# citiususc/BigSeqKit

Hardware: AMD Instinct MI355X
Metric: M records/s + GB/s (vs HBM roofline) on 100GB FASTQ stats (higher is better)
Workload: dtype u8; 1 GPU; bigseqkit stats on 100.0 GB synthetic FASTQ-150 (BASELINE C2: 315457413 records x 317 B), HBM-resident, 1 record-aligned shard(s); command=stats, records=315457413, bytes=99999999921, seed=42

## Files before the change

bigseqkit_amd/_lib.py:

```python
import ctypes as C
import os

_HERE = os.path.dirname(os.path.abspath(__file__))
LIB_PATH = os.environ.get("BSK_LIB", os.path.join(_HERE, "lib", "libbsk.so"))

if not os.path.exists(LIB_PATH):
    raise ImportError(
        f"libbsk.so not found at {LIB_PATH}: build it with ./build.sh "
        "(hipcc --offload-arch=gfx950); bigseqkit_amd has no CPU fallback")



def _preload_hip_runtime():
    import importlib.util
    try:
        spec = importlib.util.find_spec("torch")
    except Exception:
        spec = None
    if spec and spec.origin:
        cand = os.path.join(os.path.dirname(spec.origin), "lib", "libamdhip64.so")
        if os.path.exists(cand):
            try:
                C.CDLL(cand, mode=C.RTLD_GLOBAL)
            except OSError:
# ... 144 lines not shown
    "bsk_event_record": (_i, [_vp, _vp]),
    "bsk_event_elapsed_ms": (_i, [_vp, _vp, _p(C.c_float)]),
    "bsk_event_destroy": (_i, [_vp]),
    "bsk_selftest_regex_find": (_i, [C.c_char_p, C.c_char_p, _sz, _sz, _p(C.c_uint32), _p(C.c_uint32)]),
    "bsk_store_open": (_i, [C.c_char_p, _i, _p(_vp)]),
    "bsk_store_error": (C.c_char_p, [_vp]),
    "bsk_store_put": (_i, [_vp, _vp, _u64, _vp]),
    "bsk_store_put_host": (_i, [_vp, _u64, _vp, _sz]),
    "bsk_store_close": (_i, [_vp, _p(_u64)]),
    "bsk_run_to_store": (_i, [_vp, _vp, _sz, _i, _i64, _vp, _u64, _p(_u64), _p(_u64)]),
    "bsk_profile_enable": (_i, [_vp, _i]),
    "bsk_profile_read": (_i, [_vp, C.c_char_p, _p(C.c_double), _p(_u64)]),
    "bsk_profile_reset": (_i, [_vp]),
    "bsk_profile_dump": (_i, [_vp, C.c_char_p, _sz]),
    "bsk_selftest_scan": (_i, [_i, _p(C.c_uint32), _p(C.c_uint32)]),
    "bsk_selftest_rmdup_keys": (_i, [_vp, _p(_u64), _p(_u64), _sz, _p(_sz)]),
    "bsk_selftest_stream_read": (_i, [_vp, _sz, _i, _i, _p(C.c_float)]),
}

for _name, (_res, _args) in SIGNATURES.items():
    _f = getattr(lib, _name)
    _f.restype = _res
    _f.argtypes = _args


class BskError(RuntimeError):
    def __init__(self, code, message):
        super().__init__(message)
        self.code = code

# ... 7 lines not shown
```

bigseqkit_amd/csrc/anchor_wave_dev.hpp:

```cpp
#pragma once
#include <hip/hip_runtime.h>

#include <cstdint>

#include "anchor.hpp"

namespace bsk {
namespace wave_anchor {

__device__ __forceinline__ uint32_t first_eq16(const uint4& v, uint32_t rep) {
    const uint32_t w[4] = {v.x ^ rep, v.y ^ rep, v.z ^ rep, v.w ^ rep};
    uint32_t pos = 16u;
#pragma unroll
    for (int d = 3; d >= 0; --d) {
        const uint32_t x = w[d];
        const uint32_t z = ~(((x & 0x7F7F7F7Fu) + 0x7F7F7F7Fu) | x | 0x7F7F7F7Fu);
        if (z) pos = 4u * (uint32_t)d + (((uint32_t)__ffs((int)z) - 1u) >> 3);
    }
    return pos;
}

__device__ __forceinline__ uint64_t find_byte(const uint8_t* __restrict__ buf, uint64_t n, uint64_t from, uint8_t c) {
    const uint32_t lane = threadIdx.x & 63u;
    const uint32_t rep = 0x01010101u * c;
// ... 79 lines not shown
    if (e1 > s0 && buf[s0] == '+') return false;
    const uint64_t p0 = e1 + 1;
    if (p0 >= n || buf[p0] != '+') return false;
    const uint64_t e2 = find_byte(buf, n, p0, '\n');
    if (e2 >= n) return false;
    const uint64_t q0 = e2 + 1;
    const uint64_t e3 = find_byte(buf, n, q0, '\n');
    if (e3 - q0 != e1 - s0) return false;
    if (e3 + 1 < n) {
        const uint8_t c = buf[e3 + 1];
        if (c != '@' && c != '\n') return false;
    }
    return true;
}

__device__ __forceinline__ uint64_t find_fastq_start(const uint8_t* buf, uint64_t n, uint64_t from, uint64_t limit) {
    if (from >= n) return n;
    if (from == 0 && fastq_record_at(buf, n, 0)) return 0;
    uint64_t j = from == 0 ? find_byte(buf, n, 0, '\n') : find_byte(buf, n, from - 1, '\n');
    while (j < n) {
        if (fastq_record_at(buf, n, j + 1)) return j + 1;
        if (j >= limit) return ANCHOR_NONE;
        j = find_byte(buf, n, j + 1, '\n');
    }
    return n;
}

__device__ __forceinline__ uint64_t fastq_range_start(const uint8_t* buf, uint64_t n, uint64_t from) {
    const uint64_t a = find_fastq_start(buf, n, from, from + ANCHOR_SEARCH_BYTES);
    return a == ANCHOR_NONE ? from : a;
}

__device__ __forceinline__ uint64_t effective_end(const uint8_t* __restrict__ buf, uint64_t n) {
    const uint32_t lane = threadIdx.x & 63u;
    uint64_t k = 0;
    while (k < n) {
        const uint64_t left = n - k;
        const bool nl = lane < left && buf[left - 1u - lane] == '\n';
        const uint64_t other = ~__ballot(nl);
        const uint32_t run = other ? (uint32_t)__ffsll((long long)other) - 1u : 64u;
        k += run;
        if (run < 64u) break;
    }
    if (k > n) k = n;
    if (k == n) return 0;
// ... 6 lines not shown
```

bigseqkit_amd/csrc/capi.cpp:

```cpp
#include <hip/hip_runtime_api.h>

#include <algorithm>
#include <cstdio>
#include <cstdlib>
#include <cstring>
#include <new>
#include <optional>

#include "../../include/bsk.h"
#include "anchor.hpp"
#include "ctx.hpp"
#include "ops_host.hpp"
#include "ops_host_internal.hpp"
#include "ops_sample.hpp"
#include "ops_segcopy.hpp"
#include "stats_host.hpp"
#include "stream_stats.hpp"
#include "regex_vm.hpp"
#include "synth.hpp"

namespace bsk {
hipError_t launch_synth(int kind, uint64_t seed, unsigned flags, uint64_t first_record, uint8_t* dst, uint64_t n,
                        hipStream_t st);
}
// ... 398 lines not shown
    return BSK_OK;
}

static int stats_run_device(bsk_ctx* c, const uint8_t* d_buf, size_t n, int format, uint64_t* d_vec, hipStream_t st) {
    const bool fastq = format == BSK_FORMAT_FASTQ;
    const bool all = c->opts.b("All");
    const bool variant = fastq ? c->stats_a_dense : c->tune.is("stats_fasta", "events");
    const int per_cu = stats_max_blocks_per_cu(fastq, all, c->use_dpp, variant);
    const int blocks = std::max(1, c->num_cus * per_cu);
    const uint64_t waves = (uint64_t)blocks * 4;
    const uint64_t nr = pick_nranges(n, waves, c->min_range_bytes, (int)c->tune.num("ranges_per_wave"));
    const uint32_t nranges = (uint32_t)nr;
    uint64_t chunk = (n + nranges - 1) / nranges;
    chunk = (chunk + 15) & ~(uint64_t)15;
    const bool self_anchor = fastq && !all && c->use_dpp && !c->tune.is("stats_prep", "pass");
    uint32_t tickets = nranges, nsplit = nranges;
    if (self_anchor) {
        chunk = (chunk + 63) & ~(uint64_t)63;
        const uint64_t tail = nranges / 16, small = chunk / 4;
        const uint64_t floor_bytes = std::max<uint64_t>(c->min_range_bytes, (uint64_t)c->tune.num("stats_tail", 192 << 10));
        if (tail && small >= floor_bytes && !c->tune.is("stats_tail", "uniform") && (uint64_t)(nranges - tail) * chunk < n) {
            nsplit = (uint32_t)(nranges - tail);
            tickets = nsplit + (uint32_t)((n - (uint64_t)nsplit * chunk + small - 1) / small);
        }
    } else {
        int rc = ensure_range_arrays(c, nranges);
        if (rc != BSK_OK) return rc;
    }
    const uint64_t need = n / c->hist_cap + 1024;
    if (need > c->overflow_cap) {
        uint64_t* nb = nullptr;
        HIP_TRY(c, hipMalloc((void**)&nb, need * sizeof(uint64_t)));
        if (c->d_overflow) {
            HIP_TRY(c, hipMemcpyAsync(nb, c->d_overflow, c->overflow_cap * sizeof(uint64_t), hipMemcpyDeviceToDevice, st));
            HIP_TRY(c, hipStreamSynchronize(st));
            HIP_TRY(c, hipFree(c->d_overflow));
        }
        c->d_overflow = nb;
        c->overflow_cap = need;
// ... 26 lines not shown
    uint32_t* queue = self_anchor ? reinterpret_cast<uint32_t*>(c->d_ctl + bsk_ctx::CTL_STATS_QUEUE) : range_queue(c, nranges);
    D.r_head = D.r_tail = nullptr;
    D.r_flags = nullptr;
    if (!fastq) {
        if (nranges > c->rng_cap || !c->d_rng) {
            if (c->d_rng) HIP_TRY(c, hipFree(c->d_rng));
            c->d_rng = nullptr;
            HIP_TRY(c, hipMalloc((void**)&c->d_rng, (size_t)nranges * 20 + 64));
            c->rng_cap = nranges;
        }
        D.r_head = c->d_rng;
        D.r_tail = c->d_rng + nranges;
        D.r_flags = reinterpret_cast<uint32_t*>(c->d_rng + 2 * (size_t)nranges);
        HIP_TRY(c, hipMemsetAsync(c->d_rng, 0, (size_t)nranges * 20, st));
    }
    if (!self_anchor) {
        Timed t(c, "k_prep", st);
        HIP_TRY(c, launch_prep(fastq, d_buf, n, chunk, nranges, anchors, queue, st, !fastq,
                               fastq ? nullptr : c->d_anchors + (size_t)nranges + 2));
    }
    {
        Timed t(c, "k_stats", st);
        HIP_TRY(c, launch_stats(fastq, all, c->use_dpp, blocks, d_buf, n, anchors, tickets, queue, D, st, variant,
                                !fastq ? chunk : 0, self_anchor ? chunk : 0, nsplit));
    }
    if (!fastq) HIP_TRY(c, launch_stats_stitch(nranges, D, st));
    if (all && (int)gap_letters.size() > MAX_GAP_LETTERS) {
        const int rci = build_index(c, d_buf, n, format, st);
        if (rci != BSK_OK) return rci;
        uint32_t set[8] = {0, 0, 0, 0, 0, 0, 0, 0};
        for (char ch : gap_letters) set[(uint8_t)ch >> 5] |= 1u << ((uint8_t)ch & 31u);
        HIP_TRY(c, launch_gap_set_count(d_buf, c->table, set, fastq, D.vec + 2, st));
    }
    return BSK_OK;
}

static int stage_shard(bsk_ctx* c, const void* shard, size_t n, int on_device, hipStream_t st, const uint8_t** d);

int bsk_stats_run(bsk_ctx* c, const void* shard, size_t n, int on_device, int format, int64_t pid, void* d_vec,
                  void* stream) {
// ... 972 lines not shown
        HIP_TRY(nullptr, hipEventRecord(a, nullptr));
        HIP_TRY(nullptr, launch_stream_read(blocks, (const uint8_t*)d_buf, n, chunk, (uint32_t)nr, d, d + 1, nullptr));
        HIP_TRY(nullptr, hipEventRecord(b, nullptr));
        HIP_TRY(nullptr, hipEventSynchronize(b));
        float ms = 0;
        HIP_TRY(nullptr, hipEventElapsedTime(&ms, a, b));
        if (r > 0) total += ms;
    }
    *avg_ms = total / reps;
    hipEventDestroy(a);
    hipEventDestroy(b);
    hipFree(d);
    return BSK_OK;
}

int bsk_selftest_scan(int use_dpp, const uint32_t* in64, uint32_t* out64) {
    uint32_t *d_in = nullptr, *d_out = nullptr;
    HIP_TRY(nullptr, hipMalloc((void**)&d_in, 64 * 4));
    HIP_TRY(nullptr, hipMalloc((void**)&d_out, 64 * 4));
    HIP_TRY(nullptr, hipMemcpy(d_in, in64, 64 * 4, hipMemcpyHostToDevice));
    HIP_TRY(nullptr, launch_scan_selftest(use_dpp != 0, d_in, d_out, nullptr));
    HIP_TRY(nullptr, hipMemcpy(out64, d_out, 64 * 4, hipMemcpyDeviceToHost));
    hipFree(d_in);
    hipFree(d_out);
    return BSK_OK;
}

int bsk_selftest_regex_find(const char* expr, const uint8_t* text, size_t n, size_t from, uint32_t* caps4, uint32_t* ngroups) {
    try {
        const VmProgram P = compile_vm(expr ? expr : "");
// ... 10 lines not shown
```

bigseqkit_amd/csrc/stream_stats.hip:

```cpp
#include <hip/hip_runtime.h>

#include <algorithm>
#include <cstdint>

#include "anchor.hpp"
#include "anchor_wave_dev.hpp"
#include "index.hpp"
#include "stream_core_dev.hpp"
#include "stream_fasta2_dev.hpp"
#include "stream_stats.hpp"

namespace bsk {

namespace {

using namespace stream;

constexpr int BIG_SLOTS = 64;
constexpr uint32_t BIG_EMPTY = 0xFFFFFFFFu;

__device__ __forceinline__ void add_big(uint32_t len, uint32_t c, uint32_t* s_hist, const StatsDev& D) {
    uint32_t* keys = s_hist + LDS_HIST;
    uint32_t* cnts = keys + BIG_SLOTS;
    const uint32_t slot = (len * 2654435761u) >> 26;
// ... 279 lines not shown
                any_event = true;
            }
        }
    }
};

#ifndef BSK_STATS_WAVES
#define BSK_STATS_WAVES 7
#endif
#ifndef BSK_STATS_WAVES_ALL
#define BSK_STATS_WAVES_ALL 5
#endif
#ifndef BSK_STATS_WAVES_FQ
#define BSK_STATS_WAVES_FQ 6
#endif
#if BSK_STATS_WAVES
#ifndef BSK_STATS_WAVES_FA_ALL
#define BSK_STATS_WAVES_FA_ALL 5
#endif
#define BSK_STATS_ATTR __attribute__((amdgpu_waves_per_eu((ALL && FASTQ) ? BSK_STATS_WAVES_ALL : (FASTQ ? BSK_STATS_WAVES_FQ : ((ALL && ROLES_T) ? BSK_STATS_WAVES_FA_ALL : BSK_STATS_WAVES)), 8)))
#else
#define BSK_STATS_ATTR
#endif

template <bool FASTQ, bool ALL, bool DPP, bool ROLES_T = true>
__global__ __launch_bounds__(WAVES_PER_BLOCK * WAVE) BSK_STATS_ATTR void k_stats(const uint8_t* __restrict__ buf, uint64_t n,
                                                                   const uint64_t* __restrict__ anchors,
                                                                   uint32_t nranges, uint32_t* __restrict__ queue,
                                                                   StatsDev D, uint64_t chunk, uint32_t nsplit) {
    __shared__ uint32_t s_hist[LDS_HIST + 2 * BIG_SLOTS];
    constexpr bool ROLES = FASTQ && ALL && ROLES_T;
    constexpr bool SALL = ALL && !ROLES;
    constexpr int WINDOW = (FASTQ && !SALL) ? 256 : CAP;
    constexpr bool F2 = !FASTQ && ROLES_T;
    __shared__ Lds<FASTQ, SALL, F2 ? 4 : WINDOW> s_l[F2 ? 1 : WAVES_PER_BLOCK];
    __shared__ LdsF2T<F2 && ALL> s_f2[F2 ? WAVES_PER_BLOCK : 1];
    for (int i = threadIdx.x; i < LDS_HIST + 2 * BIG_SLOTS; i += blockDim.x)
        s_hist[i] = (i >= LDS_HIST && i < LDS_HIST + BIG_SLOTS) ? BIG_EMPTY : 0u;
    __syncthreads();

    const int lane = threadIdx.x & 63;
    const int wave = threadIdx.x >> 6;
    Lds<FASTQ, SALL, F2 ? 4 : WINDOW>& L = s_l[F2 ? 0 : wave];
    StatsSinkT<ROLES> sink;
    sink.s_hist = s_hist;
    sink.D = D;
    constexpr bool SELF = FASTQ && !ALL && DPP;
    const bool self_anchor = SELF && anchors == nullptr;
    const uint64_t n_eff = self_anchor ? wave_anchor::effective_end(buf, n) : anchors[nranges];
    uint64_t w20 = 0, w30 = 0, wgap = 0;
    for (;;) {
        uint32_t r = 0;
        if (lane == 0) r = atomicAdd(queue, 1u);
        r = wave_first(r);
        if (r >= nranges) break;
        uint64_t rs = 0, re = n_eff;
        if (self_anchor) {
            if constexpr (SELF) {
#pragma nounroll
                for (uint32_t k = 0; k < 2u; ++k) {
                    const uint32_t t = r + k;
                    if (t == 0u || t >= nranges) continue;
                    const uint64_t from = t <= nsplit ? (uint64_t)t * chunk : (uint64_t)nsplit * chunk + (uint64_t)(t - nsplit) * (chunk >> 2);
                    uint32_t flo = (uint32_t)from, fhi = (uint32_t)(from >> 32);
                    asm volatile("" : "+v"(flo), "+v"(fhi));
                    const uint64_t av = wave_anchor::fastq_range_start(buf, n, ((uint64_t)fhi << 32) | flo);
                    const uint64_t a = ((uint64_t)wave_first((uint32_t)(av >> 32)) << 32) | wave_first((uint32_t)av);
                    if (k == 0u) rs = a;
                    else re = a;
                }
            }
        } else {
            rs = anchors[r];
            re = anchors[r + 1];
        }
        rs = rs < n_eff ? rs : n_eff;
        re = re < n_eff ? re : n_eff;
        if (rs >= re) {
            if constexpr (!FASTQ && ALL) {
                if (chunk && r > 0u) {
                    const uint64_t lo = (uint64_t)r * chunk, hi = lo + chunk < n_eff ? lo + chunk : n_eff;
                    if (lo < hi) {
                        uint64_t cnt = 0;
                        for (uint64_t i = lo + (uint64_t)lane * 16u; i < hi; i += 64u * 16u) {
                            const uint4 v = load16(buf, hi, i);
                            for (int k = 0; k < D.pred.ngap; ++k) {
                                const uint32_t rep = D.pred.gap_rep[k];
                                if (rep == 0u && i + 16u > hi) continue;
                                cnt += popc4(zero_bytes(v.x ^ rep), zero_bytes(v.y ^ rep), zero_bytes(v.z ^ rep), zero_bytes(v.w ^ rep));
                            }
                        }
                        cnt = wave_sum_u64(cnt);
// ... 19 lines not shown
                sink.rgap = 0; sink.rsub = 0;
            }
            (void)L;
        } else {
            stream_range<FASTQ, SALL, DPP>(L, buf, n, rs, re, re == n_eff, D.pred, sink, skip_from, count_resume);
        }
        if constexpr (!FASTQ) sink.template end_range<ALL>();
        if constexpr (ROLES) {
            const uint64_t s20 = wave_sum_u64(sink.rq20), s30 = wave_sum_u64(sink.rq30), sgap = wave_sum_u64(sink.rgap);
            w20 += ((uint64_t)wave_first((uint32_t)(s20 >> 32)) << 32) | wave_first((uint32_t)s20);
            w30 += ((uint64_t)wave_first((uint32_t)(s30 >> 32)) << 32) | wave_first((uint32_t)s30);
            wgap += ((uint64_t)wave_first((uint32_t)(sgap >> 32)) << 32) | wave_first((uint32_t)sgap);
            sink.rq20 = sink.rq30 = sink.rgap = 0;
        }
    }
    if (self_anchor && lane == 0) {
        if (atomicAdd(queue + 1, 1u) == gridDim.x * (uint32_t)WAVES_PER_BLOCK - 1u) {
            atomicExch(queue + 1, 0u);
            atomicExch(queue, 0u);
        }
    }
    const uint64_t q20 = ROLES ? w20 : wave_sum_u64(sink.q20), q30 = ROLES ? w30 : wave_sum_u64(sink.q30),
                   gap = ROLES ? wgap : wave_sum_u64(sink.gap);
    const uint64_t nrec = wave_sum_u64(sink.nrec), sumlen = wave_sum_u64(sink.sumlen);
    const uint32_t err = wave_or_u32(sink.err);
    if (lane == 0) {
        if (q20) atomicAdd((unsigned long long*)&D.vec[0], (unsigned long long)q20);
        if (q30) atomicAdd((unsigned long long*)&D.vec[1], (unsigned long long)q30);
        if (gap) atomicAdd((unsigned long long*)&D.vec[2], (unsigned long long)gap);
        if (nrec) atomicAdd((unsigned long long*)&D.vec[3], (unsigned long long)nrec);
// ... 19 lines not shown
    if (r > nranges) return;
    if (r == 0) {
        if (lane0) { anchors[0] = 0; *queue = 0; }
        return;
    }
    if (r == nranges) {
        if (lane0) anchors[nranges] = effective_end(buf, n);
        return;
    }
    const uint64_t from = (uint64_t)r * chunk;
    if (!FASTQ && line_mode == 2) {
        const uint64_t a = wave_anchor::find_line_start_within(buf, n, from, from + chunk);
        if (lane0) anchors[r] = a;
        return;
    }
    const uint64_t a = FASTQ ? wave_anchor::fastq_range_start(buf, n, from)
                             : (line_mode ? wave_anchor::find_line_start(buf, n, from) : wave_anchor::find_fasta_start(buf, n, from));
    if (lane0) anchors[r] = a == ANCHOR_NONE ? from : a;
}

__global__ __launch_bounds__(256) void k_prep_fill(const uint64_t* __restrict__ raw, uint32_t nranges, uint64_t* __restrict__ anchors) {
    const uint32_t r = blockIdx.x * blockDim.x + threadIdx.x;
    if (r > nranges) return;
    uint32_t j = r;
    while (j < nranges && raw[j] == ANCHOR_NONE) ++j;
    anchors[r] = raw[j];
}

__global__ __launch_bounds__(256) void k_stats_stitch(uint32_t nranges, StatsDev D) {
    __shared__ uint32_t s_hist[LDS_HIST + 2 * BIG_SLOTS];
    __shared__ unsigned long long s_nrec, s_sum;
// ... 58 lines not shown
                if (idx + 16 <= re) {
                    const uint4 v = *reinterpret_cast<const uint4*>(buf + idx);
                    acc ^= v.x ^ v.y ^ v.z ^ v.w;
                }
            }
        }
    }
    if (acc == 0x9E3779B9u) sink[0] = acc;
}

template <bool DPP>
__global__ void k_scan_selftest(const uint32_t* in, uint32_t* out) {
    out[threadIdx.x] = wave_incl_scan<DPP>(in[threadIdx.x]);
}

}

hipError_t launch_prep(bool fastq, const uint8_t* buf, uint64_t n, uint64_t chunk, uint32_t nranges,
                       uint64_t* anchors, uint32_t* queue, hipStream_t st, bool line_mode, uint64_t* raw) {
    const int threads = 256;
    const int blocks = (int)(((uint64_t)nranges + 1 + 3) / 4);
    if (fastq) hipLaunchKernelGGL(k_prep<true>, dim3(blocks), dim3(threads), 0, st, buf, n, chunk, nranges, anchors, queue, 0);
    else if (line_mode && raw) {
        hipLaunchKernelGGL(k_prep<false>, dim3(blocks), dim3(threads), 0, st, buf, n, chunk, nranges, raw, queue, 2);
        hipLaunchKernelGGL(k_prep_fill, dim3((nranges + 1 + 255) / 256), dim3(256), 0, st, (const uint64_t*)raw, nranges, anchors);
    } else hipLaunchKernelGGL(k_prep<false>, dim3(blocks), dim3(threads), 0, st, buf, n, chunk, nranges, anchors, queue, line_mode ? 1 : 0);
    return hipGetLastError();
}

__global__ __launch_bounds__(1024) void k_stats_pack(const uint64_t* __restrict__ vec, uint32_t cap, const uint64_t* __restrict__ status,
// ... 52 lines not shown
    if (t.n == 0) return hipSuccess;
    GapSet S;
    for (int i = 0; i < 8; ++i) S.w[i] = set[i];
    const uint64_t blocks = std::min<uint64_t>((t.n + 3) / 4, 256ull * 32ull);
    hipLaunchKernelGGL(k_gap_set_count, dim3((unsigned)blocks), dim3(256), 0, st, buf, t, S, fastq ? 1 : 0, (unsigned long long*)gap_slot);
    return hipGetLastError();
}

hipError_t launch_stats_stitch(uint32_t nranges, const StatsDev& D, hipStream_t st) {
    hipLaunchKernelGGL(k_stats_stitch, dim3((nranges + 255u) / 256u), dim3(256), 0, st, nranges, D);
    return hipGetLastError();
}

template <bool FASTQ, bool ALL, bool ROLES_T = true>
static hipError_t launch_stats_t(bool dpp, int blocks, const uint8_t* buf, uint64_t n, const uint64_t* anchors,
                                 uint32_t nranges, uint32_t* queue, const StatsDev& D, hipStream_t st, uint64_t chunk, uint32_t nsplit = 0) {
    const dim3 b(WAVES_PER_BLOCK * WAVE);
    if (dpp) hipLaunchKernelGGL((k_stats<FASTQ, ALL, true, ROLES_T>), dim3(blocks), b, 0, st, buf, n, anchors, nranges, queue, D, chunk, nsplit);
    else hipLaunchKernelGGL((k_stats<FASTQ, ALL, false, ROLES_T>), dim3(blocks), b, 0, st, buf, n, anchors, nranges, queue, D, chunk, nsplit);
    return hipGetLastError();
}

hipError_t launch_stats(bool fastq, bool all, bool dpp, int blocks, const uint8_t* buf, uint64_t n,
                        const uint64_t* anchors, uint32_t nranges, uint32_t* queue, const StatsDev& D,
                        hipStream_t st, bool a_dense, uint64_t skip_chunk, uint64_t fq_chunk, uint32_t fq_nsplit) {
    if (fastq && all && a_dense) return launch_stats_t<true, true, false>(dpp, blocks, buf, n, anchors, nranges, queue, D, st, fq_chunk, fq_nsplit);
    if (fastq) return all ? launch_stats_t<true, true>(dpp, blocks, buf, n, anchors, nranges, queue, D, st, fq_chunk, fq_nsplit)
                          : launch_stats_t<true, false>(dpp, blocks, buf, n, anchors, nranges, queue, D, st, fq_chunk, fq_nsplit);
    if (all) return a_dense ? launch_stats_t<false, true, false>(dpp, blocks, buf, n, anchors, nranges, queue, D, st, skip_chunk)
                            : launch_stats_t<false, true>(dpp, blocks, buf, n, anchors, nranges, queue, D, st, skip_chunk);
    return a_dense ? launch_stats_t<false, false, false>(dpp, blocks, buf, n, anchors, nranges, queue, D, st, skip_chunk)
                   : launch_stats_t<false, false>(dpp, blocks, buf, n, anchors, nranges, queue, D, st, skip_chunk);
}

int stats_max_blocks_per_cu(bool fastq, bool all, bool dpp, bool a_dense) {
    const void* f = nullptr;
#define BSK_PICK(FQ, AL, RO)                                                            \
    f = dpp ? (const void*)k_stats<FQ, AL, true, RO> : (const void*)k_stats<FQ, AL, false, RO>;
    if (fastq && all && a_dense) { BSK_PICK(true, true, false) }
    else if (fastq && all) { BSK_PICK(true, true, true) }
    else if (fastq) { BSK_PICK(true, false, true) }
    else if (all && a_dense) { BSK_PICK(false, true, false) }
    else if (all) { BSK_PICK(false, true, true) }
    else if (a_dense) { BSK_PICK(false, false, false) }
    else { BSK_PICK(false, false, true) }
#undef BSK_PICK
    return blocks_per_cu(f, WAVES_PER_BLOCK * WAVE);
}

hipError_t launch_stream_read(int blocks, const uint8_t* buf, uint64_t n, uint64_t chunk, uint32_t nranges,
                              uint32_t* queue, uint32_t* sink, hipStream_t st) {
    hipLaunchKernelGGL(k_stream_read, dim3(blocks), dim3(WAVES_PER_BLOCK * WAVE), 0, st, buf, n, chunk, nranges, queue,
                       sink);
    return hipGetLastError();
}

hipError_t launch_scan_selftest(bool dpp, const uint32_t* in, uint32_t* out, hipStream_t st) {
    if (dpp) hipLaunchKernelGGL(k_scan_selftest<true>, dim3(1), dim3(64), 0, st, in, out);
    else hipLaunchKernelGGL(k_scan_selftest<false>, dim3(1), dim3(64), 0, st, in, out);
    return hipGetLastError();
}

}
```

bigseqkit_amd/csrc/stream_stats.hpp:

```cpp
#pragma once
#include <hip/hip_runtime_api.h>

#include <cstdint>

namespace bsk {

constexpr int STATS_HDR = 8;
constexpr int MAX_GAP_LETTERS = 8;

constexpr uint32_t ERR_BAD_HEADER = 1u;
constexpr uint32_t ERR_BAD_PLUS = 2u;
constexpr uint32_t ERR_LEN_MISMATCH = 4u;
constexpr uint32_t ERR_TRUNCATED = 8u;
constexpr uint32_t ERR_ANCHOR = 16u;
constexpr uint32_t ERR_LINE_TOO_LONG = 32u;
constexpr uint32_t ERR_CAPACITY = 64u;

inline int blocks_per_cu(const void* kernel, int threads) {
    int nb = 0;
    if (hipOccupancyMaxActiveBlocksPerMultiprocessor(&nb, kernel, threads, 0) != hipSuccess || nb < 1) nb = 1;
    return nb;
}

struct PredConsts {
// ... 16 lines not shown
};

constexpr uint32_t RF_VISITED = 1u, RF_HAS_HEADER = 2u, RF_HEAD_CLOSED = 4u, RF_TAIL_OPEN = 8u;
constexpr uint32_t RF_MID = 16u, RF_SKIP_SEQ = 32u;

hipError_t launch_prep(bool fastq, const uint8_t* buf, uint64_t n, uint64_t chunk, uint32_t nranges,
                       uint64_t* anchors, uint32_t* queue, hipStream_t st, bool line_mode = false, uint64_t* raw = nullptr);
hipError_t launch_stats_stitch(uint32_t nranges, const StatsDev& D, hipStream_t st);
struct RecordTable;
hipError_t launch_gap_set_count(const uint8_t* buf, const RecordTable& t, const uint32_t (&set)[8], bool fastq, uint64_t* gap_slot,
                                hipStream_t st);
hipError_t launch_stats_pack(const uint64_t* vec, uint32_t cap, const uint64_t* status, uint64_t* pack, uint32_t kbins, hipStream_t st);
hipError_t launch_stats(bool fastq, bool all, bool dpp, int blocks, const uint8_t* buf, uint64_t n,
                        const uint64_t* anchors, uint32_t nranges, uint32_t* queue, const StatsDev& D,
                        hipStream_t st, bool a_dense = false, uint64_t skip_chunk = 0,
                        uint64_t fq_chunk = 0, uint32_t fq_nsplit = 0);
int stats_max_blocks_per_cu(bool fastq, bool all, bool dpp, bool a_dense = false);
hipError_t launch_stream_read(int blocks, const uint8_t* buf, uint64_t n, uint64_t chunk, uint32_t nranges,
                              uint32_t* queue, uint32_t* sink, hipStream_t st);
hipError_t launch_scan_selftest(bool dpp, const uint32_t* in, uint32_t* out, hipStream_t st);

}
```

include/bsk.h:

```cpp
#ifndef BSK_H
#define BSK_H

#include <stddef.h>
#include <stdint.h>

#ifdef __cplusplus
extern "C" {
#endif

#define BSK_OK 0
#define BSK_ERR_INVALID_ARG 1
#define BSK_ERR_OPTS 2
#define BSK_ERR_FORMAT 3
#define BSK_ERR_UNSUPPORTED 4
#define BSK_ERR_HIP 5
#define BSK_ERR_NO_DEVICE 6
#define BSK_ERR_CAPACITY 7
#define BSK_ERR_OVERFLOW_EXCHANGE 8

#define BSK_FORMAT_FASTA 0
#define BSK_FORMAT_FASTQ 1

typedef struct bsk_ctx bsk_ctx;

// ... 202 lines not shown
uint64_t bsk_synth_offset(int kind, uint64_t record);
int bsk_synth_host(int kind, uint64_t seed, unsigned flags, uint64_t first_record, uint8_t* dst, size_t n);
int bsk_synth_device(int kind, uint64_t seed, unsigned flags, uint64_t first_record, void* d_dst, size_t n, int device,
                     void* stream);

int bsk_event_create(void** ev);
int bsk_event_record(void* ev, void* stream);
int bsk_event_elapsed_ms(void* start, void* stop, float* ms);
int bsk_event_destroy(void* ev);
int bsk_profile_enable(bsk_ctx* ctx, int on);
int bsk_profile_read(bsk_ctx* ctx, const char* kernel, double* total_ms, uint64_t* launches);
int bsk_profile_reset(bsk_ctx* ctx);
int bsk_profile_dump(bsk_ctx* ctx, char* buf, size_t cap);

int bsk_selftest_scan(int use_dpp, const uint32_t* in64, uint32_t* out64);
int bsk_selftest_rmdup_keys(bsk_ctx* ctx, uint64_t* k1, uint64_t* k2, size_t cap, size_t* n_out);
int bsk_selftest_stream_read(const void* d_buf, size_t n, int reps, int blocks_per_cu, float* avg_ms);

#ifdef __cplusplus
}
#endif
#endif
```

Before: 20950 M records/s.

## Use geometric multi-level tail ranges and windowed FASTQ anchor search in stats

Replaces the single split of the stats work queue (uniform chunks plus one small-chunk tail) with up to eight levels of halving range sizes, each ticket mapped to its boundary through a per-level table passed as a kernel argument. Self-anchoring FASTQ range starts now load a 2 KB window per wave once, build newline/@/+ bitmasks across lanes, and validate record starts from those masks, falling back to the byte scan only when the window is inconclusive. The aim is better tail load balance and fewer dependent global loads when finding record boundaries. In exchange the kernel carries more argument state and branching, and adds optional clock instrumentation and selftests.

Result: no change. 20910 M records/s (-0.2%).

```diff
diff --git a/bigseqkit_amd/_lib.py b/bigseqkit_amd/_lib.py
--- a/bigseqkit_amd/_lib.py
+++ b/bigseqkit_amd/_lib.py
@@ -182,6 +182,9 @@
     "bsk_profile_reset": (_i, [_vp]),
     "bsk_profile_dump": (_i, [_vp, C.c_char_p, _sz]),
     "bsk_selftest_scan": (_i, [_i, _p(C.c_uint32), _p(C.c_uint32)]),
+    "bsk_selftest_fastq_range_start": (_i, [C.c_void_p, C.c_size_t, _p(C.c_uint64), C.c_size_t, C.c_size_t, _p(C.c_uint64)]),
+    "bsk_selftest_fastq_range_start_host": (_i, [C.c_void_p, C.c_size_t, _p(C.c_uint64), C.c_size_t, _i, _p(C.c_uint64)]),
+    "bsk_selftest_stats_levels": (_i, [C.c_uint64, C.c_uint64, C.c_uint64, _i, C.c_uint64, _p(C.c_uint64), _p(C.c_uint64)]),
     "bsk_selftest_rmdup_keys": (_i, [_vp, _p(_u64), _p(_u64), _sz, _p(_sz)]),
     "bsk_selftest_stream_read": (_i, [_vp, _sz, _i, _i, _p(C.c_float)]),
 }
diff --git a/bigseqkit_amd/csrc/anchor_wave_dev.hpp b/bigseqkit_amd/csrc/anchor_wave_dev.hpp
--- a/bigseqkit_amd/csrc/anchor_wave_dev.hpp
+++ b/bigseqkit_amd/csrc/anchor_wave_dev.hpp
@@ -117,10 +117,8 @@
     return true;
 }
 
-__device__ __forceinline__ uint64_t find_fastq_start(const uint8_t* buf, uint64_t n, uint64_t from, uint64_t limit) {
-    if (from >= n) return n;
-    if (from == 0 && fastq_record_at(buf, n, 0)) return 0;
-    uint64_t j = from == 0 ? find_byte(buf, n, 0, '\n') : find_byte(buf, n, from - 1, '\n');
+__device__ __forceinline__ uint64_t find_fastq_start_from(const uint8_t* buf, uint64_t n, uint64_t x, uint64_t limit) {
+    uint64_t j = find_byte(buf, n, x, '\n');
     while (j < n) {
         if (fastq_record_at(buf, n, j + 1)) return j + 1;
         if (j >= limit) return ANCHOR_NONE;
@@ -129,9 +127,143 @@
     return n;
 }
 
+__device__ __forceinline__ uint64_t find_fastq_start(const uint8_t* buf, uint64_t n, uint64_t from, uint64_t limit) {
+    if (from >= n) return n;
+    if (from == 0 && fastq_record_at(buf, n, 0)) return 0;
+    return find_fastq_start_from(buf, n, from == 0 ? 0 : from - 1, limit);
+}
+
 __device__ __forceinline__ uint64_t fastq_range_start(const uint8_t* buf, uint64_t n, uint64_t from) {
     const uint64_t a = find_fastq_start(buf, n, from, from + ANCHOR_SEARCH_BYTES);
     return a == ANCHOR_NONE ? from : a;
+}
+
+constexpr uint32_t WIN_BYTES = 2048u;
+constexpr uint32_t WIN_NONE = 0xFFFFFFFFu;
+
+struct FqWindow { uint32_t nl, at, pl; };
+
+__device__ __forceinline__ uint64_t fastq_window_base(const uint8_t* buf, uint64_t from) {
+    const uint64_t x = from - 1u;
+    const uint64_t off = (uint64_t)(reinterpret_cast<uintptr_t>(buf + x) & 15u);
+    return x >= off ? x - off : x;
+}
+
+__device__ __forceinline__ uint4 window_load16(const uint8_t* __restrict__ buf, uint64_t n, uint64_t i) {
+    uint4 v = make_uint4(0u, 0u, 0u, 0u);
+    if (i + 16u <= n) __builtin_memcpy(&v, buf + i, 16);
+    else if (i < n) {
+        uint32_t w[4] = {0u, 0u, 0u, 0u};
+        for (uint32_t b = 0; b < 16u && i + b < n; ++b) w[b >> 2] |= (uint32_t)buf[i + b] << ((b & 3u) * 8u);
+        v = make_uint4(w[0], w[1], w[2], w[3]);
+    }
+    return v;
+}
+
+__device__ __forceinline__ void fastq_window_load(const uint8_t* __restrict__ buf, uint64_t n, uint64_t w0, uint4& a, uint4& b) {
+    const uint64_t i = w0 + (uint64_t)(threadIdx.x & 63u) * 32u;
+    a = window_load16(buf, n, i);
+    b = window_load16(buf, n, i + 16u);
+}
+
+__device__ __forceinline__ uint32_t window_eq16(const uint4& v, uint32_t rep) {
+    const uint32_t w[4] = {v.x ^ rep, v.y ^ rep, v.z ^ rep, v.w ^ rep};
+    uint32_t m = 0u;
+#pragma unroll
+    for (int d = 0; d < 4; ++d) {
+        const uint32_t x = w[d];
+        const uint32_t z = ~(((x & 0x7F7F7F7Fu) + 0x7F7F7F7Fu) | x | 0x7F7F7F7Fu);
+        m |= (((z >> 7) | (z >> 14) | (z >> 21) | (z >> 28)) & 0xFu) << (4 * d);
+    }
+    return m;
+}
+
+__device__ __forceinline__ FqWindow fastq_window_masks(const uint4& a, const uint4& b) {
+    FqWindow W;
+    W.nl = window_eq16(a, 0x0A0A0A0Au) | (window_eq16(b, 0x0A0A0A0Au) << 16);
+    W.at = window_eq16(a, 0x40404040u) | (window_eq16(b, 0x40404040u) << 16);
+    W.pl = window_eq16(a, 0x2B2B2B2Bu) | (window_eq16(b, 0x2B2B2B2Bu) << 16);
+    return W;
+}
+
+__device__ __forceinline__ uint32_t window_next(uint32_t m, uint64_t any, uint32_t x) {
+    if (x >= WIN_BYTES) return WIN_NONE;
+    const uint32_t l = x >> 5;
+    const uint32_t w = (uint32_t)__builtin_amdgcn_readlane((int)m, (int)l) & (~0u << (x & 31u));
+    if (w) return (l << 5) + (uint32_t)__ffs((int)w) - 1u;
+    const uint64_t rest = l >= 63u ? 0ull : any & (~0ull << (l + 1u));
+    if (!rest) return WIN_NONE;
+    const uint32_t l2 = (uint32_t)__ffsll((long long)rest) - 1u;
+    return (l2 << 5) + (uint32_t)__ffs(__builtin_amdgcn_readlane((int)m, (int)l2)) - 1u;
+}
+__device__ __forceinline__ bool window_bit(uint32_t m, uint32_t x) {
+    return (((uint32_t)__builtin_amdgcn_readlane((int)m, (int)(x >> 5)) >> (x & 31u)) & 1u) != 0u;
+}
+
+__device__ __forceinline__ int fastq_window_record_at(const FqWindow& W, uint64_t any_nl, uint32_t p, uint32_t end) {
+    const bool reach = end != WIN_NONE;
+    const int open = reach ? 0 : -1;
+    if (reach && p >= end) return 0;
+    if (p >= WIN_BYTES) return -1;
+    if (!window_bit(W.at, p)) return 0;
+    const uint32_t e0 = window_next(W.nl, any_nl, p);
+    if (e0 == WIN_NONE) return open;
+    const uint32_t s0 = e0 + 1u;
+    const uint32_t e1 = window_next(W.nl, any_nl, s0);
+    if (e1 == WIN_NONE) return open;
+    if (e1 > s0 && window_bit(W.pl, s0)) return 0;
+    const uint32_t p0 = e1 + 1u;
+    if (reach && p0 >= end) return 0;
+    if (p0 >= WIN_BYTES) return -1;
+    if (!window_bit(W.pl, p0)) return 0;
+    const uint32_t e2 = window_next(W.nl, any_nl, p0);
+    if (e2 == WIN_NONE) return open;
+    const uint32_t q0 = e2 + 1u;
+    uint32_t e3 = window_next(W.nl, any_nl, q0);
+    if (e3 == WIN_NONE) {
+        if (!reach) return -1;
+        e3 = end;
+    }
+    if (e3 - q0 != e1 - s0) return 0;
+    const uint32_t f = e3 + 1u;
+    if (reach && f >= end) return 1;
+    if (f >= WIN_BYTES) return -1;
+    return (window_bit(W.at, f) || window_bit(W.nl, f)) ? 1 : 0;
+}
+
+__device__ __forceinline__ bool fastq_window_search(const FqWindow& W, uint64_t w0, uint64_t n, uint64_t from, uint64_t& out) {
+    const uint64_t left = n - w0;
+    const uint32_t end = left <= (uint64_t)WIN_BYTES ? (uint32_t)left : WIN_NONE;
+    const uint64_t any_nl = __ballot(W.nl != 0u);
+    uint32_t x = (uint32_t)(from - 1u - w0);
+    for (;;) {
+        const uint32_t j = window_next(W.nl, any_nl, x);
+        if (j == WIN_NONE) {
+            if (end != WIN_NONE) { out = n; return true; }
+            out = w0 + x;
+            return false;
+        }
+        const int v = fastq_window_record_at(W, any_nl, j + 1u, end);
+        if (v > 0) { out = w0 + j + 1u; return true; }
+        if (v < 0) { out = w0 + j; return false; }
+        x = j + 1u;
+    }
+}
+
+__device__ __forceinline__ uint64_t fastq_range_start_resume(const uint8_t* buf, uint64_t n, uint64_t from, uint64_t resume) {
+    const uint64_t a = find_fastq_start_from(buf, n, resume, from + ANCHOR_SEARCH_BYTES);
+    return a == ANCHOR_NONE ? from : a;
+}
+
+__device__ __forceinline__ uint64_t fastq_range_start_window(const uint8_t* buf, uint64_t n, uint64_t from) {
+    if (from == 0 || from >= n) return fastq_range_start(buf, n, from);
+    const uint64_t w0 = fastq_window_base(buf, from);
+    uint4 a, b;
+    fastq_window_load(buf, n, w0, a, b);
+    const FqWindow W = fastq_window_masks(a, b);
+    uint64_t out;
+    if (fastq_window_search(W, w0, n, from, out)) return out;
+    return fastq_range_start_resume(buf, n, from, out);
 }
 
 __device__ __forceinline__ uint64_t effective_end(const uint8_t* __restrict__ buf, uint64_t n) {
diff --git a/bigseqkit_amd/csrc/capi.cpp b/bigseqkit_amd/csrc/capi.cpp
--- a/bigseqkit_amd/csrc/capi.cpp
+++ b/bigseqkit_amd/csrc/capi.cpp
@@ -436,15 +436,15 @@
     uint64_t chunk = (n + nranges - 1) / nranges;
     chunk = (chunk + 15) & ~(uint64_t)15;
     const bool self_anchor = fastq && !all && c->use_dpp && !c->tune.is("stats_prep", "pass");
-    uint32_t tickets = nranges, nsplit = nranges;
+    uint32_t tickets = nranges;
+    StatsLevels levels;
     if (self_anchor) {
-        chunk = (chunk + 63) & ~(uint64_t)63;
-        const uint64_t tail = nranges / 16, small = chunk / 4;
-        const uint64_t floor_bytes = std::max<uint64_t>(c->min_range_bytes, (uint64_t)c->tune.num("stats_tail", 192 << 10));
-        if (tail && small >= floor_bytes && !c->tune.is("stats_tail", "uniform") && (uint64_t)(nranges - tail) * chunk < n) {
-            nsplit = (uint32_t)(nranges - tail);
-            tickets = nsplit + (uint32_t)((n - (uint64_t)nsplit * chunk + small - 1) / small);
-        }
+        const uint64_t floor_bytes = c->tune.is("stats_tail", "uniform") ? 0
+                                     : c->tune.get("stats_tail") ? std::max<uint64_t>(16, (uint64_t)c->tune.num("stats_tail", 0))
+                                                                 : std::max<uint64_t>(c->min_range_bytes, STATS_TAIL_FLOOR);
+        const uint64_t t = stats_build_levels(n, chunk, nranges, waves, floor_bytes, levels);
+        if (t > 0xFFFFFFFEull) return fail(c, BSK_ERR_CAPACITY, "libbsk: stats: too many ranges");
+        tickets = (uint32_t)t;
     } else {
         int rc = ensure_range_arrays(c, nranges);
         if (rc != BSK_OK) return rc;
@@ -501,6 +501,15 @@
         D.r_flags = reinterpret_cast<uint32_t*>(c->d_rng + 2 * (size_t)nranges);
         HIP_TRY(c, hipMemsetAsync(c->d_rng, 0, (size_t)nranges * 20, st));
     }
+#if defined(BSK_STATS_CLOCKS) && BSK_STATS_CLOCKS
+    static uint64_t* d_clk = nullptr;
+    const size_t clk_bytes = (size_t)waves * 64 * sizeof(uint64_t);
+    if (self_anchor && getenv("BSK_STATS_CLOCKS_OUT")) {
+        if (!d_clk) HIP_TRY(c, hipMalloc((void**)&d_clk, clk_bytes));
+        HIP_TRY(c, hipMemsetAsync(d_clk, 0, clk_bytes, st));
+        D.r_tail = d_clk;
+    }
+#endif
     if (!self_anchor) {
         Timed t(c, "k_prep", st);
         HIP_TRY(c, launch_prep(fastq, d_buf, n, chunk, nranges, anchors, queue, st, !fastq,
@@ -509,8 +518,16 @@
     {
         Timed t(c, "k_stats", st);
         HIP_TRY(c, launch_stats(fastq, all, c->use_dpp, blocks, d_buf, n, anchors, tickets, queue, D, st, variant,
-                                !fastq ? chunk : 0, self_anchor ? chunk : 0, nsplit));
-    }
+                                !fastq ? chunk : 0, self_anchor ? chunk : 0, self_anchor ? &levels : nullptr));
+    }
+#if defined(BSK_STATS_CLOCKS) && BSK_STATS_CLOCKS
+    if (self_anchor && D.r_tail) {
+        std::vector<uint64_t> h((size_t)waves * 64);
+        HIP_TRY(c, hipStreamSynchronize(st));
+        HIP_TRY(c, hipMemcpy(h.data(), d_clk, clk_bytes, hipMemcpyDeviceToHost));
+        if (FILE* f = fopen(getenv("BSK_STATS_CLOCKS_OUT"), "wb")) { fwrite(h.data(), 8, h.size(), f); fclose(f); }
+    }
+#endif
     if (!fastq) HIP_TRY(c, launch_stats_stitch(nranges, D, st));
     if (all && (int)gap_letters.size() > MAX_GAP_LETTERS) {
         const int rci = build_index(c, d_buf, n, format, st);
@@ -1513,6 +1530,58 @@
     return BSK_OK;
 }
 
+int bsk_selftest_stats_levels(uint64_t n, uint64_t waves, uint64_t min_range_bytes, int ranges_per_wave, uint64_t floor_bytes,
+                              uint64_t* out25, uint64_t* tickets) {
+    if (!out25 || !tickets || n == 0) return fail_global(BSK_ERR_INVALID_ARG, "libbsk: null argument");
+    if (waves == 0) {
+        hipDeviceProp_t p;
+        HIP_TRY(nullptr, hipGetDeviceProperties(&p, 0));
+        waves = (uint64_t)std::max(1, p.multiProcessorCount * stats_max_blocks_per_cu(true, false, true, false)) * 4;
+    }
+    const uint64_t nranges = pick_nranges(n, waves, min_range_bytes, ranges_per_wave);
+    uint64_t chunk = (n + nranges - 1) / nranges;
+    chunk = (chunk + 15) & ~(uint64_t)15;
+    StatsLevels L;
+    *tickets = stats_build_levels(n, chunk, nranges, waves, floor_bytes, L);
+    out25[0] = L.nlev;
+    for (int i = 0; i < STATS_MAX_LEVELS; ++i) {
+        const bool on = (uint32_t)i < L.nlev;
+        out25[1 + 3 * i] = on ? L.t0[i] : 0;
+        out25[2 + 3 * i] = on ? L.b0[i] : 0;
+        out25[3 + 3 * i] = on ? L.size[i] : 0;
+    }
+    return BSK_OK;
+}
+
+int bsk_selftest_fastq_range_start_host(const uint8_t* text, size_t n, const uint64_t* from, size_t count, int which, uint64_t* out) {
+    if (!text || !from || !out) return fail_global(BSK_ERR_INVALID_ARG, "libbsk: null argument");
+    for (size_t i = 0; i < count; ++i) {
+        if (which == 0) out[i] = find_fastq_cut(text, n, from[i]);
+        else {
+            const uint64_t a = find_fastq_start(text, n, from[i], from[i] + ANCHOR_SEARCH_BYTES);
+            out[i] = a == ANCHOR_NONE ? from[i] : a;
+        }
+    }
+    return BSK_OK;
+}
+
+int bsk_selftest_fastq_range_start(const uint8_t* text, size_t n, const uint64_t* from, size_t count, size_t view_offset, uint64_t* out) {
+    if (!text || !from || !out || n == 0 || count == 0) return fail_global(BSK_ERR_INVALID_ARG, "libbsk: null argument");
+    uint8_t* d_buf = nullptr;
+    uint64_t *d_from = nullptr, *d_out = nullptr;
+    HIP_TRY(nullptr, hipMalloc((void**)&d_buf, n + view_offset));
+    HIP_TRY(nullptr, hipMalloc((void**)&d_from, count * 8));
+    HIP_TRY(nullptr, hipMalloc((void**)&d_out, count * 8));
+    HIP_TRY(nullptr, hipMemcpy(d_buf + view_offset, text, n, hipMemcpyHostToDevice));
+    HIP_TRY(nullptr, hipMemcpy(d_from, from, count * 8, hipMemcpyHostToDevice));
+    HIP_TRY(nullptr, launch_range_start_selftest(d_buf + view_offset, n, d_from, count, d_out, nullptr));
+    HIP_TRY(nullptr, hipMemcpy(out, d_out, count * 8, hipMemcpyDeviceToHost));
+    hipFree(d_buf);
+    hipFree(d_from);
+    hipFree(d_out);
+    return BSK_OK;
+}
+
 int bsk_selftest_scan(int use_dpp, const uint32_t* in64, uint32_t* out64) {
     uint32_t *d_in = nullptr, *d_out = nullptr;
     HIP_TRY(nullptr, hipMalloc((void**)&d_in, 64 * 4));
diff --git a/bigseqkit_amd/csrc/stats_levels.hpp b/bigseqkit_amd/csrc/stats_levels.hpp
--- /dev/null
+++ b/bigseqkit_amd/csrc/stats_levels.hpp
@@ -0,0 +1,61 @@
+#pragma once
+#include <algorithm>
+#include <cstdint>
+
+namespace bsk {
+
+constexpr int STATS_MAX_LEVELS = 8;
+
+struct StatsLevels {
+    uint32_t nlev;
+    uint32_t t0[STATS_MAX_LEVELS];
+    uint64_t b0[STATS_MAX_LEVELS];
+    uint64_t size[STATS_MAX_LEVELS];
+};
+
+inline uint64_t stats_level_boundary(const StatsLevels& L, uint64_t t) {
+    uint32_t i = 0;
+    while (i + 1u < L.nlev && t >= L.t0[i + 1u]) ++i;
+    return L.b0[i] + (t - L.t0[i]) * L.size[i];
+}
+
+inline uint64_t stats_build_levels(uint64_t n, uint64_t chunk, uint64_t nranges, uint64_t waves, uint64_t floor_bytes, StatsLevels& L) {
+    L.nlev = 0;
+    for (int i = 0; i < STATS_MAX_LEVELS; ++i) { L.t0[i] = 0xFFFFFFFFu; L.b0[i] = 0; L.size[i] = 0; }
+    chunk = std::max<uint64_t>(16, (chunk + 15) & ~(uint64_t)15);
+    uint64_t sz[STATS_MAX_LEVELS];
+    int k = 0;
+    sz[0] = chunk;
+    const uint64_t per_level = std::min<uint64_t>(waves, nranges / 4);
+    uint64_t tail_bytes = 0;
+    if (floor_bytes && per_level) {
+        floor_bytes = std::max<uint64_t>(16, floor_bytes);
+        while (k + 1 < STATS_MAX_LEVELS) {
+            const uint64_t half = (((sz[k] + 1) / 2) + 15) & ~(uint64_t)15;
+            if (half < floor_bytes || half >= sz[k]) break;
+            sz[++k] = half;
+            tail_bytes += per_level * half;
+        }
+        if (tail_bytes >= n) { k = 0; tail_bytes = 0; }
+    }
+    uint64_t t = 0, b = 0;
+    for (int i = 0; i <= k && b < n; ++i) {
+        const uint64_t left = (n - b + sz[i] - 1) / sz[i];
+        const uint64_t want = i == k ? left : (i == 0 ? (n - tail_bytes + chunk - 1) / chunk : per_level);
+        const uint64_t cnt = std::min(want, left);
+        if (cnt == 0) continue;
+        L.t0[L.nlev] = (uint32_t)std::min<uint64_t>(t, 0xFFFFFFFFull);
+        L.b0[L.nlev] = b;
+        L.size[L.nlev] = sz[i];
+        ++L.nlev;
+        t += cnt;
+        b += cnt * sz[i];
+    }
+    if (L.nlev == 0) {
+        L.nlev = 1; L.t0[0] = 0; L.b0[0] = 0; L.size[0] = chunk;
+        t = 1;
+    }
+    return t;
+}
+
+}
diff --git a/bigseqkit_amd/csrc/stream_stats.hip b/bigseqkit_amd/csrc/stream_stats.hip
--- a/bigseqkit_amd/csrc/stream_stats.hip
+++ b/bigseqkit_amd/csrc/stream_stats.hip
@@ -317,6 +317,9 @@
 #ifndef BSK_STATS_WAVES_FQ
 #define BSK_STATS_WAVES_FQ 6
 #endif
+#ifndef BSK_STATS_CLOCKS
+#define BSK_STATS_CLOCKS 0
+#endif
 #if BSK_STATS_WAVES
 #ifndef BSK_STATS_WAVES_FA_ALL
 #define BSK_STATS_WAVES_FA_ALL 5
@@ -325,12 +328,26 @@
 #else
 #define BSK_STATS_ATTR
 #endif
+
+struct KStatsArgs {
+    const uint8_t* buf; uint64_t n; const uint64_t* anchors; uint32_t nranges; uint32_t* queue; StatsDev D; uint64_t chunk; StatsLevels lv;
+};
+
+__device__ __forceinline__ uint64_t ticket_boundary(uint32_t t, uint32_t& lvl) {
+    constexpr uint32_t LV = (uint32_t)offsetof(KStatsArgs, lv);
+#pragma nounroll
+    while (lvl + 1u < (uint32_t)STATS_MAX_LEVELS && t >= karg_load<uint32_t>(LV + (uint32_t)offsetof(StatsLevels, t0) + 4u * (lvl + 1u))) ++lvl;
+    const uint32_t t0 = karg_load<uint32_t>(LV + (uint32_t)offsetof(StatsLevels, t0) + 4u * lvl);
+    const uint64_t b0 = karg_load<uint64_t>(LV + (uint32_t)offsetof(StatsLevels, b0) + 8u * lvl);
+    const uint64_t sz = karg_load<uint64_t>(LV + (uint32_t)offsetof(StatsLevels, size) + 8u * lvl);
+    return b0 + (uint64_t)(t - t0) * sz;
+}
 
 template <bool FASTQ, bool ALL, bool DPP, bool ROLES_T = true>
 __global__ __launch_bounds__(WAVES_PER_BLOCK * WAVE) BSK_STATS_ATTR void k_stats(const uint8_t* __restrict__ buf, uint64_t n,
                                                                    const uint64_t* __restrict__ anchors,
                                                                    uint32_t nranges, uint32_t* __restrict__ queue,
-                                                                   StatsDev D, uint64_t chunk, uint32_t nsplit) {
+                                                                   StatsDev D, uint64_t chunk, StatsLevels lv) {
     __shared__ uint32_t s_hist[LDS_HIST + 2 * BIG_SLOTS];
     constexpr bool ROLES = FASTQ && ALL && ROLES_T;
     constexpr bool SALL = ALL && !ROLES;
@@ -350,25 +367,51 @@
     sink.D = D;
     constexpr bool SELF = FASTQ && !ALL && DPP;
     const bool self_anchor = SELF && anchors == nullptr;
+#if BSK_STATS_CLOCKS
+    uint64_t* const clk = (SELF && D.r_tail) ? D.r_tail + 64u * ((uint64_t)blockIdx.x * WAVES_PER_BLOCK + (uint32_t)wave) : nullptr;
+    uint32_t clk_n = 0;
+    if (clk && lane == 0) clk[0] = wall_clock64();
+#endif
     const uint64_t n_eff = self_anchor ? wave_anchor::effective_end(buf, n) : anchors[nranges];
+#if BSK_STATS_CLOCKS
+    if (clk && lane == 0) clk[62] = wall_clock64();
+#endif
     uint64_t w20 = 0, w30 = 0, wgap = 0;
     for (;;) {
         uint32_t r = 0;
         if (lane == 0) r = atomicAdd(queue, 1u);
         r = wave_first(r);
+#if BSK_STATS_CLOCKS
+        if (clk && lane == 0 && clk_n < 29u) clk[4u + 2u * clk_n] = wall_clock64();
+#endif
         if (r >= nranges) break;
         uint64_t rs = 0, re = n_eff;
         if (self_anchor) {
             if constexpr (SELF) {
+                uint32_t lvl = 0;
+                const uint64_t f0 = r != 0u ? ticket_boundary(r, lvl) : 0ull;
+                const uint64_t f1 = r + 1u < nranges ? ticket_boundary(r + 1u, lvl) : n;
+                const bool on0 = f0 != 0ull && f0 < n, on1 = f1 < n;
+                const uint64_t w0 = on0 ? wave_anchor::fastq_window_base(buf, f0) : 0ull;
+                const uint64_t w1 = on1 ? wave_anchor::fastq_window_base(buf, f1) : 0ull;
+                uint4 a0, b0, a1, b1;
+                wave_anchor::fastq_window_load(buf, on0 ? n : 0ull, w0, a0, b0);
+                wave_anchor::fastq_window_load(buf, on1 ? n : 0ull, w1, a1, b1);
+                const wave_anchor::FqWindow W0 = wave_anchor::fastq_window_masks(a0, b0), W1 = wave_anchor::fastq_window_masks(a1, b1);
+                if (f0 >= n) rs = n;
 #pragma nounroll
                 for (uint32_t k = 0; k < 2u; ++k) {
-                    const uint32_t t = r + k;
-                    if (t == 0u || t >= nranges) continue;
-                    const uint64_t from = t <= nsplit ? (uint64_t)t * chunk : (uint64_t)nsplit * chunk + (uint64_t)(t - nsplit) * (chunk >> 2);
-                    uint32_t flo = (uint32_t)from, fhi = (uint32_t)(from >> 32);
-                    asm volatile("" : "+v"(flo), "+v"(fhi));
-                    const uint64_t av = wave_anchor::fastq_range_start(buf, n, ((uint64_t)fhi << 32) | flo);
-                    const uint64_t a = ((uint64_t)wave_first((uint32_t)(av >> 32)) << 32) | wave_first((uint32_t)av);
+                    if (!(k ? on1 : on0)) continue;
+                    wave_anchor::FqWindow W;
+                    W.nl = k ? W1.nl : W0.nl; W.at = k ? W1.at : W0.at; W.pl = k ? W1.pl : W0.pl;
+                    const uint64_t from = k ? f1 : f0;
+                    uint64_t a;
+                    if (!wave_anchor::fastq_window_search(W, k ? w1 : w0, n, from, a)) {
+                        uint32_t xlo = (uint32_t)a, xhi = (uint32_t)(a >> 32);
+                        asm volatile("" : "+v"(xlo), "+v"(xhi));
+                        const uint64_t av = wave_anchor::fastq_range_start_resume(buf, n, from, ((uint64_t)xhi << 32) | xlo);
+                        a = ((uint64_t)wave_first((uint32_t)(av >> 32)) << 32) | wave_first((uint32_t)av);
+                    }
                     if (k == 0u) rs = a;
                     else re = a;
                 }
@@ -379,6 +422,17 @@
         }
         rs = rs < n_eff ? rs : n_eff;
         re = re < n_eff ? re : n_eff;
+#if BSK_STATS_CLOCKS
+        if (clk && lane == 0) {
+            if (clk_n < 29u) clk[5u + 2u * clk_n] = wall_clock64();
+            if (clk_n == 0u && rs < re) {
+                const uint8_t first = *reinterpret_cast<const volatile uint8_t*>(buf + rs);
+                asm volatile("s_waitcnt vmcnt(0)" ::"v"((uint32_t)first) : "memory");
+                clk[2] = wall_clock64();
+            }
+        }
+        ++clk_n;
+#endif
         if (rs >= re) {
             if constexpr (!FASTQ && ALL) {
                 if (chunk && r > 0u) {
@@ -428,6 +482,9 @@
             sink.rq20 = sink.rq30 = sink.rgap = 0;
         }
     }
+#if BSK_STATS_CLOCKS
+    if (clk && lane == 0) { clk[1] = clk_n; clk[3] = wall_clock64(); }
+#endif
     if (self_anchor && lane == 0) {
         if (atomicAdd(queue + 1, 1u) == gridDim.x * (uint32_t)WAVES_PER_BLOCK - 1u) {
             atomicExch(queue + 1, 0u);
@@ -477,7 +534,7 @@
         if (lane0) anchors[r] = a;
         return;
     }
-    const uint64_t a = FASTQ ? wave_anchor::fastq_range_start(buf, n, from)
+    const uint64_t a = FASTQ ? wave_anchor::fastq_range_start_window(buf, n, from)
                              : (line_mode ? wave_anchor::find_line_start(buf, n, from) : wave_anchor::find_fasta_start(buf, n, from));
     if (lane0) anchors[r] = a == ANCHOR_NONE ? from : a;
 }
@@ -566,6 +623,14 @@
     out[threadIdx.x] = wave_incl_scan<DPP>(in[threadIdx.x]);
 }
 
+__global__ __launch_bounds__(256) void k_range_start_selftest(const uint8_t* __restrict__ buf, uint64_t n, const uint64_t* __restrict__ from,
+                                                              uint64_t count, uint64_t* __restrict__ out) {
+    const uint64_t i = (uint64_t)blockIdx.x * (blockDim.x >> 6) + (threadIdx.x >> 6);
+    if (i >= count) return;
+    const uint64_t a = wave_anchor::fastq_range_start_window(buf, n, from[i]);
+    if ((threadIdx.x & 63u) == 0u) out[i] = a;
+}
+
 }
 
 hipError_t launch_prep(bool fastq, const uint8_t* buf, uint64_t n, uint64_t chunk, uint32_t nranges,
@@ -648,19 +713,20 @@
 
 template <bool FASTQ, bool ALL, bool ROLES_T = true>
 static hipError_t launch_stats_t(bool dpp, int blocks, const uint8_t* buf, uint64_t n, const uint64_t* anchors,
-                                 uint32_t nranges, uint32_t* queue, const StatsDev& D, hipStream_t st, uint64_t chunk, uint32_t nsplit = 0) {
+                                 uint32_t nranges, uint32_t* queue, const StatsDev& D, hipStream_t st, uint64_t chunk, const StatsLevels& lv = StatsLevels{}) {
     const dim3 b(WAVES_PER_BLOCK * WAVE);
-    if (dpp) hipLaunchKernelGGL((k_stats<FASTQ, ALL, true, ROLES_T>), dim3(blocks), b, 0, st, buf, n, anchors, nranges, queue, D, chunk, nsplit);
-    else hipLaunchKernelGGL((k_stats<FASTQ, ALL, false, ROLES_T>), dim3(blocks), b, 0, st, buf, n, anchors, nranges, queue, D, chunk, nsplit);
+    if (dpp) hipLaunchKernelGGL((k_stats<FASTQ, ALL, true, ROLES_T>), dim3(blocks), b, 0, st, buf, n, anchors, nranges, queue, D, chunk, lv);
+    else hipLaunchKernelGGL((k_stats<FASTQ, ALL, false, ROLES_T>), dim3(blocks), b, 0, st, buf, n, anchors, nranges, queue, D, chunk, lv);
     return hipGetLastError();
 }
 
 hipError_t launch_stats(bool fastq, bool all, bool dpp, int blocks, const uint8_t* buf, uint64_t n,
                         const uint64_t* anchors, uint32_t nranges, uint32_t* queue, const StatsDev& D,
-                        hipStream_t st, bool a_dense, uint64_t skip_chunk, uint64_t fq_chunk, uint32_t fq_nsplit) {
-    if (fastq && all && a_dense) return launch_stats_t<true, true, false>(dpp, blocks, buf, n, anchors, nranges, queue, D, st, fq_chunk, fq_nsplit);
-    if (fastq) return all ? launch_stats_t<true, true>(dpp, blocks, buf, n, anchors, nranges, queue, D, st, fq_chunk, fq_nsplit)
-                          : launch_stats_t<true, false>(dpp, blocks, buf, n, anchors, nranges, queue, D, st, fq_chunk, fq_nsplit);
+                        hipStream_t st, bool a_dense, uint64_t skip_chunk, uint64_t fq_chunk, const StatsLevels* fq_levels) {
+    const StatsLevels fq_lv = fq_levels ? *fq_levels : StatsLevels{};
+    if (fastq && all && a_dense) return launch_stats_t<true, true, false>(dpp, blocks, buf, n, anchors, nranges, queue, D, st, fq_chunk, fq_lv);
+    if (fastq) return all ? launch_stats_t<true, true>(dpp, blocks, buf, n, anchors, nranges, queue, D, st, fq_chunk, fq_lv)
+                          : launch_stats_t<true, false>(dpp, blocks, buf, n, anchors, nranges, queue, D, st, fq_chunk, fq_lv);
     if (all) return a_dense ? launch_stats_t<false, true, false>(dpp, blocks, buf, n, anchors, nranges, queue, D, st, skip_chunk)
                             : launch_stats_t<false, true>(dpp, blocks, buf, n, anchors, nranges, queue, D, st, skip_chunk);
     return a_dense ? launch_stats_t<false, false, false>(dpp, blocks, buf, n, anchors, nranges, queue, D, st, skip_chunk)
@@ -689,6 +755,11 @@
     return hipGetLastError();
 }
 
+hipError_t launch_range_start_selftest(const uint8_t* buf, uint64_t n, const uint64_t* from, uint64_t count, uint64_t* out, hipStream_t st) {
+    hipLaunchKernelGGL(k_range_start_selftest, dim3((unsigned)((count + 3) / 4)), dim3(256), 0, st, buf, n, from, count, out);
+    return hipGetLastError();
+}
+
 hipError_t launch_scan_selftest(bool dpp, const uint32_t* in, uint32_t* out, hipStream_t st) {
     if (dpp) hipLaunchKernelGGL(k_scan_selftest<true>, dim3(1), dim3(64), 0, st, in, out);
     else hipLaunchKernelGGL(k_scan_selftest<false>, dim3(1), dim3(64), 0, st, in, out);
diff --git a/bigseqkit_amd/csrc/stream_stats.hpp b/bigseqkit_amd/csrc/stream_stats.hpp
--- a/bigseqkit_amd/csrc/stream_stats.hpp
+++ b/bigseqkit_amd/csrc/stream_stats.hpp
@@ -3,10 +3,13 @@
 
 #include <cstdint>
 
+#include "stats_levels.hpp"
+
 namespace bsk {
 
 constexpr int STATS_HDR = 8;
 constexpr int MAX_GAP_LETTERS = 8;
+constexpr uint64_t STATS_TAIL_FLOOR = 192 << 10;
 
 constexpr uint32_t ERR_BAD_HEADER = 1u;
 constexpr uint32_t ERR_BAD_PLUS = 2u;
@@ -54,10 +57,11 @@
 hipError_t launch_stats(bool fastq, bool all, bool dpp, int blocks, const uint8_t* buf, uint64_t n,
                         const uint64_t* anchors, uint32_t nranges, uint32_t* queue, const StatsDev& D,
                         hipStream_t st, bool a_dense = false, uint64_t skip_chunk = 0,
-                        uint64_t fq_chunk = 0, uint32_t fq_nsplit = 0);
+                        uint64_t fq_chunk = 0, const StatsLevels* fq_levels = nullptr);
 int stats_max_blocks_per_cu(bool fastq, bool all, bool dpp, bool a_dense = false);
 hipError_t launch_stream_read(int blocks, const uint8_t* buf, uint64_t n, uint64_t chunk, uint32_t nranges,
                               uint32_t* queue, uint32_t* sink, hipStream_t st);
 hipError_t launch_scan_selftest(bool dpp, const uint32_t* in, uint32_t* out, hipStream_t st);
+hipError_t launch_range_start_selftest(const uint8_t* buf, uint64_t n, const uint64_t* from, uint64_t count, uint64_t* out, hipStream_t st);
 
 }
diff --git a/include/bsk.h b/include/bsk.h
--- a/include/bsk.h
+++ b/include/bsk.h
@@ -240,6 +240,10 @@
 int bsk_profile_dump(bsk_ctx* ctx, char* buf, size_t cap);
 
 int bsk_selftest_scan(int use_dpp, const uint32_t* in64, uint32_t* out64);
+int bsk_selftest_fastq_range_start(const uint8_t* text, size_t n, const uint64_t* from, size_t count, size_t view_offset, uint64_t* out);
+int bsk_selftest_fastq_range_start_host(const uint8_t* text, size_t n, const uint64_t* from, size_t count, int which, uint64_t* out);
+int bsk_selftest_stats_levels(uint64_t n, uint64_t waves, uint64_t min_range_bytes, int ranges_per_wave, uint64_t floor_bytes,
+                              uint64_t* out25, uint64_t* tickets);
 int bsk_selftest_rmdup_keys(bsk_ctx* ctx, uint64_t* k1, uint64_t* k2, size_t cap, size_t* n_out);
 int bsk_selftest_stream_read(const void* d_buf, size_t n, int reps, int blocks_per_cu, float* avg_ms);
 
```
